# davelailai/DS-GCN

Hardware: AMD Instinct MI355X
Metric: clips/sec fwd+bwd, DS-STGCN NTU-60 3x64x25x2 (higher is better)
Workload: dtype f32; 1 GPU; DS-STGCN configs/dsstgcn/ntu60_xsub_3dkp/j.py (DSSTGCN_model.py kwargs), 64 clips/GPU of 3x64x25x2, 60 classes, train-mode BN, CE loss, fwd+bwd+grad all-reduce+SGD-nesterov per step; clips_per_gpu=64, global_batch=64, parallelism=dp1

## Files before the change

ds-gcn_amd/kernels.py:

```python
import contextlib
import sys

_active = None


def ops():
    return _active if _active is not None else sys.modules[__name__]


@contextlib.contextmanager
def use_ops(namespace):
    global _active
    prev = _active
    _active = namespace
    try:
        yield namespace
    finally:
        _active = prev


NAME = 'hip'

import torch

# ... 1394 lines not shown
    return KT or 3, types, c0s, bcs, dils, ws, bs


class _TemporalFused(torch.autograd.Function):

    @staticmethod
    def forward(ctx, z, zaug, scale, shift, coeff, gamma, beta, n_act, stride, KT, types, c0s, bcs, dils, eps, want_bn,
                bn, *wb):
        _require_cuda(z)
        ctx.bn, ctx.bn_in = bn, _bn_of(scale)
        z, zaug, scale, shift, coeff, gamma, beta = [_f32c(t) for t in (z, zaug, scale, shift, coeff, gamma, beta)]
        nbr = len(types)
        ws = [_f32c(t) for t in wb[:nbr]]
        bs = [_f32c(t) for t in wb[nbr:]]
        n, C, T, V = z.shape
        Tout = (T + stride - 1) // stride
        dev = z.device
        lib = native.lib()
        aug = zaug is not None
        tabs = (_int_array(types), _int_array(c0s), _int_array(bcs), _int_array(dils))
        rows = lib.dsgcn_tms_rows(0, n, C, T, V, stride, KT, nbr, tabs[0], tabs[2], tabs[3], int(aug))
        assert rows > 0
        f = torch.empty((n, C, Tout, V), device=dev, dtype=torch.float32)
        oaug = torch.empty((n, C, Tout), device=dev, dtype=torch.float32) if aug else None
        stats = torch.empty((rows, C, 2), device=dev, dtype=torch.float32) if want_bn else None
        rc = lib.dsgcn_tms_fwd(_ptr(z), _ptr(zaug), _ptr(scale), _ptr(shift), int(n_act), _ptr(coeff), _ptr(f),
                               _ptr(oaug), _ptr(stats), n, C, T, V, stride, KT, nbr, *tabs, _ptr_array(ws),
                               _ptr_array(bs), _stream())
        native.check(rc, 'dsgcn_tms_fwd')
        scale1 = shift1 = mean = var = None
        count = float(n * Tout * V)
        if want_bn:
            mean, var, scale1, shift1 = _finalize_stats(ctx, stats, rows, C, count, gamma, beta, eps, C)
        ctx.set_materialize_grads(False)
        ctx.save_for_backward(z, zaug, scale, shift, coeff, f, oaug, gamma, mean, var, *[w for w in ws if w is not None])
        ctx.cfg = (int(n_act), int(stride), int(KT), tuple(types), tuple(c0s), tuple(bcs), tuple(dils), float(eps),
                   bool(want_bn), count, beta is not None, tuple(b is not None for b in bs))
        ctx.defer_ok = _leafish(coeff, *wb)
        return f, scale1, shift1, mean, var

    @staticmethod
    def backward(ctx, gf, gscale, gshift, _gm, _gv):
        z, zaug, scale, shift, coeff, f, oaug, gamma, mean, var, *wsaved = ctx.saved_tensors
        n_act, stride, KT, types, c0s, bcs, dils, eps, want_bn, count, has_beta, has_b = ctx.cfg
        n, C, T, V = z.shape
        nbr = len(types)
        dev = z.device
        lib = native.lib()
        st = _stream()
        aug = zaug is not None
        gf, gscale, gshift = _f32c(gf), _f32c(gscale), _f32c(gshift)
        A0 = B0 = dgamma = dbeta = None
        if want_bn:
            dgamma, dbeta, A0, B0 = _bn_coef(ctx.bn, gscale, gshift, mean, var, gamma, eps, count, C, C)
        if gf is None:
            gf = torch.zeros_like(f)
        it = iter(wsaved)
        ws = [next(it) if t == 0 else None for t in types]
        tabs = (_int_array(types), _int_array(c0s), _int_array(bcs), _int_array(dils))
        rows = lib.dsgcn_tms_rows(1, n, C, T, V, stride, KT, nbr, tabs[0], tabs[2], tabs[3], int(aug))
        paff = torch.empty((rows, C, 2), device=dev, dtype=torch.float32)
        pcoeff = torch.empty((rows * nbr, V), device=dev, dtype=torch.float32) if aug else None
        dz = torch.empty_like(z)
        dzaug = torch.empty_like(zaug) if aug else None
        rc = lib.dsgcn_tms_dgrad(_ptr(z), _ptr(zaug), _ptr(scale), _ptr(shift), n_act, _ptr(coeff), _ptr(gf), _ptr(f),
                                 _ptr(A0), _ptr(B0), _ptr(oaug), _ptr(dz), _ptr(dzaug), _ptr(paff), _ptr(pcoeff), n, C, T,
                                 V, stride, KT, nbr, *tabs, _ptr_array(ws), st)
        native.check(rc, 'dsgcn_tms_dgrad')
        (dscale, dshift), _ = _affine_tail(paff, 2, [(scale, ctx.bn_in, 0, 1)])
        dcoeff = param_colsum(pcoeff, ctx.defer_ok) if aug else None
        dws, dbs = [None] * nbr, [None] * nbr
        if 0 in types:
            rows2 = lib.dsgcn_tms_rows(2, n, C, T, V, stride, KT, nbr, tabs[0], tabs[2], tabs[3], int(aug))
            part, dwp, dbp, pstride, split = _branch_partials(types, bcs, bcs, KT, rows2, dev, has_b)
            rc = lib.dsgcn_tms_wgrad(_ptr(z), _ptr(zaug), _ptr(scale), _ptr(shift), n_act, _ptr(coeff), _ptr(gf), _ptr(f),
                                     _ptr(A0), _ptr(B0), n, C, T, V, stride, KT, nbr, *tabs, dwp, dbp, pstride, st)
            native.check(rc, 'dsgcn_tms_wgrad')
            dws, dbs = split(param_colsum(part, ctx.defer_ok))
        dgamma, dbeta = _trim_affine_grads(dgamma, dbeta, gamma, has_beta)
        return (dz, dzaug, dscale, dshift, dcoeff, dgamma, dbeta, None, None, None, None, None, None, None, None, None,
                None, *dws, *dbs)


class _TemporalSplit(torch.autograd.Function):
    FRONT = 32

    @staticmethod
    def forward(ctx, z, zaug, scale, shift, coeff, gamma, beta, n_act, stride, types, c0s, bcs, dils, eps, want_bn, bn, *wb):
        _require_cuda(z)
        ctx.bn = bn
        z, zaug, scale, shift, coeff, gamma, beta = [_f32c(t) for t in (z, zaug, scale, shift, coeff, gamma, beta)]
        nbr = len(types)
        ws = [_f32c(t) for t in wb[:nbr]]
        bs = [_f32c(t) for t in wb[nbr:]]
        n, C, T, V = z.shape
        To = T // stride
        dev = z.device
        lib = native.lib()
        tabs = (_int_array(types), _int_array(c0s), _int_array(bcs), _int_array(dils))
        rows = lib.dsgcn_tms_split_rows(0, n, C, T, V, stride, 3, nbr, *tabs)
        assert rows > 0
        f = torch.empty((n, C, To, V), device=dev, dtype=torch.float32)
        oaug = torch.empty((n, C, To), device=dev, dtype=torch.float32)
        stats = torch.empty((rows, C, 2), device=dev, dtype=torch.float32) if want_bn else None
        rc = lib.dsgcn_tms_split_fwd(_ptr(z), _ptr(zaug), _ptr(scale), _ptr(shift), int(n_act), _ptr(coeff), _ptr(f),
                                     _ptr(oaug), _ptr(stats), n, C, T, V, stride, nbr, *tabs, _ptr_array(ws), _ptr_array(bs),
                                     _stream())
        native.check(rc, 'dsgcn_tms_split_fwd')
        scale1 = shift1 = mean = var = None
        count = float(n * To * V)
        if want_bn:
            mean, var, scale1, shift1 = _finalize_stats(ctx, stats, rows, C, count, gamma, beta, eps, C)
        ctx.set_materialize_grads(False)
        ctx.save_for_backward(z, zaug, scale, shift, coeff, f, oaug, gamma, mean, var, *[w for w in ws if w is not None])
        ctx.cfg = (int(n_act), int(stride), tuple(types), tuple(c0s), tuple(bcs), tuple(dils), float(eps), bool(want_bn),
                   count, beta is not None, tuple(b is not None for b in bs))
        ctx.bn_in = _bn_of(scale)
        ctx.defer_ok = _leafish(coeff, *wb)
        return f, scale1, shift1, mean, var

    @staticmethod
    def backward(ctx, gf, gscale, gshift, _gm, _gv):
        z, zaug, scale, shift, coeff, f, oaug, gamma, mean, var, *wsaved = ctx.saved_tensors
        n_act, stride, types, c0s, bcs, dils, eps, want_bn, count, has_beta, has_b = ctx.cfg
        n, C, T, V = z.shape
        To = f.shape[2]
        nbr = len(types)
        dev = z.device
        lib = native.lib()
        st = _stream()
        gf, gscale, gshift = _f32c(gf), _f32c(gscale), _f32c(gshift)
        A0 = B0 = dgamma = dbeta = None
        if want_bn:
            dgamma, dbeta, A0, B0 = _bn_coef(ctx.bn, gscale, gshift, mean, var, gamma, eps, count, C, C)
        FR = _TemporalSplit.FRONT
        gbuf = torch.empty(FR + f.numel() + FR + n * C * To, device=dev, dtype=torch.float32)
        ge = gbuf[FR:FR + f.numel()].view(f.shape)
        doaug = gbuf[2 * FR + f.numel():].view(n, C, To)
        pcoef = torch.empty((n * C, V), device=dev, dtype=torch.float32)
        rc = lib.dsgcn_tms_split_prep(_ptr(gf), _ptr(f), _ptr(oaug), _ptr(coeff), _ptr(A0), _ptr(B0), _ptr(ge), _ptr(doaug),
                                      _ptr(pcoef), n, C, To, V, st)
        native.check(rc, 'dsgcn_tms_split_prep')
        dcoeff = param_colsum(pcoef, ctx.defer_ok)
        it = iter(wsaved)
        ws = [next(it) if t == 0 else None for t in types]
        tabs = (_int_array(types), _int_array(c0s), _int_array(bcs), _int_array(dils))
        rows = lib.dsgcn_tms_split_rows(1, n, C, T, V, stride, 3, nbr, *tabs)
        part = torch.empty((rows, C, 2), device=dev, dtype=torch.float32)
        dz = torch.empty_like(z)
        dzaug = torch.empty_like(zaug)
        rc = lib.dsgcn_tms_split_dgrad(_ptr(z), _ptr(zaug), _ptr(scale), _ptr(shift), n_act, _ptr(ge), _ptr(doaug), _ptr(dz),
                                       _ptr(dzaug), _ptr(part), n, C, T, V, stride, nbr, *tabs, _ptr_array(ws), st)
        native.check(rc, 'dsgcn_tms_split_dgrad')
        (dscale, dshift), hosted = _affine_tail(part, 2, [(scale, ctx.bn_in, 0, 1)], launch=False)
        splits = lib.dsgcn_tms_split_rows(2, n, C, T, V, stride, 3, nbr, *tabs)
        wpart, dwp, dbp, pstride, split = _branch_partials(types, bcs, bcs, 3, splits, dev, has_b)
        rc = lib.dsgcn_tms_split_wgrad_jobs(_ptr(z), _ptr(zaug), _ptr(scale), _ptr(shift), n_act, _ptr(ge), _ptr(doaug), n, C,
                                            T, V, stride, nbr, *tabs, dwp, dbp, splits, pstride, *_job_array(hosted), st)
        native.check(rc, 'dsgcn_tms_split_wgrad_jobs')
        dws, dbs = split(param_colsum(wpart, ctx.defer_ok))
        dgamma, dbeta = _trim_affine_grads(dgamma, dbeta, gamma, has_beta)
        return (dz, dzaug, dscale, dshift, dcoeff, dgamma, dbeta, None, None, None, None, None, None, None, None, None,
                *dws, *dbs)


def _split_temporal(z, zaug, scale, shift, coeff, n_act, branch_cfg, widths, conv_w, conv_b, stride, gamma, beta, eps,
                    want_bn):
    if zaug is None or any(not isinstance(c, str) and c[0] != 'max' and c[0] != 3 for c in branch_cfg):
        return None
    if int(stride) != 1 and SPLIT_TEMPORAL == '1':
        return None
    KT, types, c0s, bcs, dils, ws, bs = _branch_tables(branch_cfg, widths, conv_w, conv_b)
    n, C, T, V = z.shape
    if native.lib().dsgcn_tms_split_rows(-1, n, C, T, V, int(stride), KT, len(types), _int_array(types), _int_array(c0s),
                                         _int_array(bcs), _int_array(dils)) != 1:
        return None
    bn = BNCtx() if want_bn else None
    out = _TemporalSplit.apply(z, zaug, scale, shift, coeff, gamma, beta, int(n_act), int(stride), types, c0s, bcs, dils,
                               float(eps), bool(want_bn), bn, *ws, *bs)
    if want_bn:
        _bn_attach(out[1], bn, out[3], out[4], gamma, eps, float(n * (T // int(stride)) * V), C)
    return out


def _fused_temporal(z, zaug, scale, shift, coeff, n_act, branch_cfg, widths, conv_w, conv_b, stride, gamma, beta, eps,
                    want_bn):
    KT, types, c0s, bcs, dils, ws, bs = _branch_tables(branch_cfg, widths, conv_w, conv_b)
    n, C, T, V = z.shape
    if FUSED_TEMPORAL == '0' or (FUSED_TEMPORAL == 'auto' and KT == 3):
        return None
    if sum(bcs) != C or any(c0s[i] + bcs[i] != c0s[i + 1] for i in range(len(bcs) - 1)) or c0s[0] != 0:
        return None
    rows = native.lib().dsgcn_tms_rows(0, n, C, T, V, int(stride), KT, len(types), _int_array(types), _int_array(bcs),
                                       _int_array(dils), int(zaug is not None))
    if rows <= 0:
        return None
    bn = BNCtx() if want_bn else None
    out = _TemporalFused.apply(z, zaug, scale, shift, coeff, gamma, beta, int(n_act), int(stride), KT, types, c0s, bcs,
                               dils, float(eps), bool(want_bn), bn, *ws, *bs)
    if want_bn:
        Tout = (T + int(stride) - 1) // int(stride)
        _bn_attach(out[1], bn, out[3], out[4], gamma, eps, float(n * Tout * V), C)
    return out


def temporal_ms(z, zaug, scale, shift, n_act, branch_cfg, widths, conv_w, conv_b, add_coeff, stride, gamma=None,
                beta=None, eps=1e-5, want_bn=False):
    _require_cuda(z)
    n, C, T, V = z.shape
    coeff = add_coeff if add_coeff.shape[0] == V else add_coeff[:V].contiguous()
    if FUSED_TEMPORAL != '0':
        out = _fused_temporal(z, zaug, scale, shift, coeff, n_act, branch_cfg, widths, conv_w, conv_b, stride, gamma, beta,
                              eps, want_bn)
        if out is not None:
            return out
    if SPLIT_TEMPORAL != '0':
        out = _split_temporal(z, zaug, scale, shift, coeff, n_act, branch_cfg, widths, conv_w, conv_b, stride, gamma, beta,
                              eps, want_bn)
        if out is not None:
            return out
    h = _BranchAct.apply(z, zaug, scale, shift, n_act)
    KT, types, c0s, bcs, dils, ws, bs = _branch_tables(branch_cfg, widths, conv_w, conv_b)
    o = _TapBranches.apply(h, int(stride), KT, C, types, c0s, c0s, bcs, bcs, dils, *ws, *bs)
    bn = BNCtx() if want_bn else None
    out = _TmsCombine.apply(o, coeff, gamma, beta, float(eps), bool(want_bn), bn)
    if want_bn:
        _bn_attach(out[1], bn, out[3], out[4], gamma, eps, float(o.shape[0] * o.shape[2] * (o.shape[3] - 1)), o.shape[1])
    return out


class _TapBranchesZero(_TapBranches):

    @staticmethod
    def forward(ctx, *args):
        return _TapBranches._run(ctx, torch.zeros, *args)

# ... 1025 lines not shown
```

include/dsgcn.h:

```cpp
#ifndef DSGCN_H_
#define DSGCN_H_

#include <stddef.h>
#include "dsgcn_jobs.h"
#ifdef __cplusplus
extern "C" {
#endif

#define DSGCN_EINVAL (-1)
#define DSGCN_EUNSUPPORTED (-2)

int dsgcn_version(void);

int dsgcn_set_matmul_precision(int level);
int dsgcn_get_matmul_precision(void);
int dsgcn_pwconv_terms(int dir, int n, int Ci, int Co, int T, int V, int stride);
int dsgcn_tconv_terms(int dir, int n, int Ci, int Co, int T, int V, int KT, int stride);

int dsgcn_aggregate_fwd(const float* zp, const float* scale, const float* shift, int relu, const float* ahat,
                        float* y, int n, int KC, int T, int V, void* stream);

int dsgcn_aggregate_bwd_partial_rows(int n, int T, int V);
int dsgcn_aggregate_bwd(const float* zp, const float* scale, const float* shift, int relu, const float* ahat,
                        const float* dy, float* dzp, float* dahat, float* partial, int n, int KC, int T, int V,
// ... 191 lines not shown
int dsgcn_tanhdiff_fwd(const float* proj, float* d, int n, int K, int R, int V, void* stream);
int dsgcn_tanhdiff_bwd_k(const float* d, const float* const* dd, float* dproj, int n, int K, int R, int V, void* stream);
int dsgcn_tanhdiff_aug_fwd(const float* proj, const float* A, float* d, int n, int K, int R, int V, void* stream);
int dsgcn_tanhdiff_aug_bwd(const float* d, const float* const* dd, float* dproj, float* dAp, int n, int K, int R, int V,
                           void* stream);
int dsgcn_ctr_wprep_multi(const dsgcn_ctr_prep_job* jobs, int njobs, void* stream);
int dsgcn_ctr_wfin_multi(const dsgcn_ctr_fin_job* jobs, int njobs, void* stream);
int dsgcn_ctr_affine_fwd(const float* const* s, const float* alpha, int alpha_stride, const float* A, const float* beta,
                         const float* G, float* ahat, int n, int K, int Co, int V, void* stream);
int dsgcn_ctr_affine_bwd(const float* const* s, const float* alpha, int alpha_stride, const float* dahat,
                         float* const* ds, float* prow, int n, int K, int Co, int V, void* stream);
int dsgcn_edge_select_fwd(const float* in, const int* edge_type, float* out, int n, int R, int E, int V, void* stream);
int dsgcn_edge_select_bwd(const float* dout, const int* edge_type, float* din, int n, int R, int E, int V, void* stream);
int dsgcn_plane_stats(const float* x, float* partial, long planes, int L, void* stream);

#define DSGCN_TYPED_MAX_TYPES 16
#define DSGCN_TYPED_MAX_PERIOD 1024
int dsgcn_typedconv_fwd(const float* x, const float* w, const float* b, const int* plan, int ntiles, float* y, int n,
                        int Ci, int Co, int TV, int L, int chunk, int P, void* stream);
int dsgcn_typedconv_dgrad(const float* dy, const float* w, const int* plan, int ntiles, float* dx, int n, int Ci, int Co,
                          int TV, int L, int chunk, int P, void* stream);
int dsgcn_typedconv_wgrad_rows(int n, int Ci, int Co, int P);
int dsgcn_typedconv_wgrad(const float* x, const float* dy, const int* plan, int ntiles, float* part, int n, int Ci, int Co,
                          int TV, int L, int chunk, int P, void* stream);

int dsgcn_add3(const float* a, const float* b, const float* c, float* out, long n, void* stream);

int dsgcn_pack(const float* const* src_table, const long* dst_offsets, const int* numels, int count, float* dst,
               void* stream);
int dsgcn_pack_fill(const float* const* src_table, const long* dst_offsets, const long* numels, int count, float* dst,
                    void* stream);

int dsgcn_dwcausal_fwd(const float* h, const float* w, const float* b, const int* dil, float* y, int n, int C, int T,
                       int V, int stride, int KM, void* stream);
int dsgcn_dwcausal_bwd(const float* h, const float* w, const int* dil, const float* dy, float* dh, float* part, int n,
                       int C, int T, int V, int stride, int KM, void* stream);

int dsgcn_mlpwin_supported(int n, int C, int T, int V1, int stride, int KM, int nwin, const int* type, const int* c0,
                           const int* width, const int* dil, const int* add);
int dsgcn_mlpwin_partial_stride(int C, int KM, int nwin, const int* type, const int* width);
int dsgcn_mlpwin_fwd(const float* h, const float* o, float* u, const float* tapw, const float* tapb, int n, int C, int T,
                     int V1, int stride, int KM, int nwin, const int* type, const int* c0, const int* width, const int* dil,
                     const int* add, const float* const* w1, const float* const* b1, void* stream);
int dsgcn_mlpwin_bwd(const float* h, const float* o, const float* du, const float* tapw, const float* tapb, float* dh,
                     float* dout, float* gbuf, float* part, int n, int C, int T, int V1, int stride, int KM, int nwin, const int* type,
                     const int* c0, const int* width, const int* dil, const int* add, const float* const* w1, int pstride,
                     void* stream);

int dsgcn_tms_rows(int which, int n, int C, int T, int V, int stride, int KT, int nbr, const int* type, const int* bc,
                   const int* dil, int aug);
int dsgcn_tms_fwd(const float* z, const float* zaug, const float* scale, const float* shift, int n_act,
                  const float* coeff, float* f, float* oaug, float* stats, int n, int C, int T, int V, int stride, int KT,
                  int nbr, const int* type, const int* c0, const int* bc, const int* dil, const float* const* w,
                  const float* const* b, void* stream);
int dsgcn_tms_dgrad(const float* z, const float* zaug, const float* scale, const float* shift, int n_act,
                    const float* coeff, const float* gf, const float* f, const float* A0, const float* B0,
                    const float* oaug, float* dz, float* dzaug, float* paff, float* pcoeff, int n, int C, int T, int V,
                    int stride, int KT, int nbr, const int* type, const int* c0, const int* bc, const int* dil,
                    const float* const* w, void* stream);
int dsgcn_tms_wgrad(const float* z, const float* zaug, const float* scale, const float* shift, int n_act,
                    const float* coeff, const float* gf, const float* f, const float* A0, const float* B0, int n, int C,
                    int T, int V, int stride, int KT, int nbr, const int* type, const int* c0, const int* bc,
                    const int* dil, float* const* dwp, float* const* dbp, int pstride, void* stream);

int dsgcn_tms_split_rows(int which, int n, int C, int T, int V, int stride, int KT, int nbr, const int* type,
                         const int* c0, const int* bc, const int* dil);
int dsgcn_tms_split_fwd(const float* z, const float* zaug, const float* scale, const float* shift, int n_act,
                        const float* coeff, float* f, float* oaug, float* stats, int n, int C, int T, int V, int stride,
                        int nbr, const int* type, const int* c0, const int* bc, const int* dil, const float* const* w,
                        const float* const* b, void* stream);
int dsgcn_tms_split_prep(const float* gf, const float* f, const float* oaug, const float* coeff, const float* A0,
                         const float* B0, float* ge, float* doaug, float* pcoef, int n, int C, int T, int V,
                         void* stream);
int dsgcn_tms_split_dgrad(const float* z, const float* zaug, const float* scale, const float* shift, int n_act,
                          const float* ge, const float* doaug, float* dz, float* dzaug, float* part, int n, int C, int T,
                          int V, int stride, int nbr, const int* type, const int* c0, const int* bc, const int* dil,
                          const float* const* w, void* stream);
int dsgcn_tms_split_wgrad_jobs(const float* z, const float* zaug, const float* scale, const float* shift, int n_act,
                               const float* ge, const float* doaug, int n, int C, int T, int V, int stride, int nbr,
                               const int* type, const int* c0, const int* bc, const int* dil, float* const* dwp,
                               float* const* dbp, int splits, int pstride, const dsgcn_bn_coef_job* jobs, int njobs,
                               void* stream);

int dsgcn_gate_fwd(const float* y, const float* g, int mode, float* out, float* rout, int rmode, int n, int C, int T,
                   int V, void* stream);
int dsgcn_gate_bwd(const float* y, const float* g, int mode, const float* gout, const float* drout, int rmode, float* dy,
                   float* dgp, int n, int C, int T, int V, void* stream);

int dsgcn_skeleton_prep(const float* raw, const long* offset, const int* M, const int* T, const int* flags,
                        const int* f0, const int* f1, const float* center, const float* matrix, const int* parent,
                        float* out, int N, int clips, int Mout, int clip_len, int V, int C, int nfeat, int fmask,
                        int scored, int loop, void* stream);

int dsgcn_skeleton_prep_streams(const float* raw, const long* offset, const int* M, const int* T, const int* flags,
                                const int* f0, const int* f1, const float* center, const float* matrix,
                                const int* parent, float* const* out, int N, int clips, int Mout, int clip_len, int V,
                                int C, int nfeat, int fmask, int scored, int loop, void* stream);

int dsgcn_head_loss_fwd(const float* feat, const float* w, const float* b, const long long* label, int N, int M, int C,
                        int K, float loss_weight, float* pooled, float* score, float* prob, float* clip, float* loss,
                        double* acc, void* stream);
int dsgcn_head_loss_bwd(const float* prob, const float* pooled, const float* w, const long long* label, const float* gloss,
                        int N, int M, int C, int K, float loss_weight, float* dfeat, float* dw, float* db, void* stream);

int dsgcn_head_target_fwd(const float* feat, const float* w, const float* b, const float* class_weight, const void* target,
                          int mode, int N, int M, int C, int K, float loss_weight, float* pooled, float* score,
                          float* dscore, float* clip, float* loss, float* den, double* acc, void* stream);
int dsgcn_head_target_bwd(const float* dscore, const float* pooled, const float* w, const float* gloss, const float* den,
                          int N, int M, int C, int K, float loss_weight, float* dfeat, float* dw, float* db, void* stream);

int dsgcn_head_test_fwd(const float* feat, const float* w, const float* b, int N, int clips, int M, int C, int K, int mode,
                        float* clip_score, float* out, void* stream);

int dsgcn_head_ensemble_fwd(const float* const* feat, const float* const* w, const float* const* b, const float* weight,
                            int S, int N, int clips, int M, int C, int K, int mode, float* stream_out, float* out,
                            void* stream);

int dsgcn_feat_ext_fwd(const float* x, const float* w, const float* b, int videos, int clips, int M, int C, int T, int V,
                       int K, int pool_mask, float* out32, void* out16, void* stream);

int dsgcn_graph_pool_splits(int videos, int group, int K, int mid, int V);
int dsgcn_graph_pool(const float* ahat, float* out, float* ws, int videos, int group, int K, int mid, int V, int L,
                     int layer, void* stream);

int dsgcn_bn_running_multi(float* const* running_mean, float* const* running_var, const float* const* mean,
                           const float* const* var, long long* const* num_batches_tracked, const int* C,
                           const float* unbias, const float* momentum, int njobs, void* stream);

int dsgcn_data_bn_fwd(const float* x, const float* gamma, const float* beta, float* running_mean, float* running_var,
                      long long* num_batches_tracked, float* y, float* save_mean, float* save_invstd, float* scratch,
                      int N, int M, int T, int V, int C, int mvc, int training, float eps, float momentum,
                      void* stream);
int dsgcn_data_bn_bwd(const float* x, const float* dy, const float* save_mean, const float* save_invstd, float* pg,
                      float* pb, int N, int M, int T, int V, int C, int mvc, void* stream);

int dsgcn_sgd_step(float* p, const float* g, float* buf, const float* lr, float momentum, float weight_decay,
                   int nesterov, long long n, void* stream);

int dsgcn_grad_norm_rows(long long n);
int dsgcn_grad_norm_partials(const float* g, long long n, int norm_type, double* partial, void* stream);
int dsgcn_sgd_step_clip(float* p, float* g, float* buf, const float* lr, const double* partial, int rows, int norm_type,
                        float max_norm, float* grad_norm_out, float momentum, float weight_decay, int nesterov,
                        long long n, void* stream);

int dsgcn_grad_accum(float* acc, const float* g, long long n, void* stream);
int dsgcn_grad_accum_finish(float* acc, float* g, const float* factor, long long n, void* stream);

#define DSGCN_OPTIM_SKIP (-1)
int dsgcn_optim_chunks(long long n);
int dsgcn_optim_table(const int* ends, const int* group, int ntens, const double* wd, int groups, long long n, int* first);
int dsgcn_sgd_group_step(float* p, float* g, float* buf, const int* ends, const int* group, const int* first, int ntens,
                         const double* lr, const double* wd, int groups, float momentum, int nesterov, long long n,
                         void* stream);
int dsgcn_sgd_group_step_clip(float* p, float* g, float* buf, const int* ends, const int* group, const int* first, int ntens,
                              const double* lr, const double* wd, int groups, const double* partial, int rows,
                              int norm_type, float max_norm, float* grad_norm_out, float momentum, int nesterov,
                              long long n, void* stream);
int dsgcn_adam_step(float* p, float* g, float* m, float* v, int* step, const int* ends, const int* group, const int* first,
                    int ntens, const double* lr, const double* wd, int groups, double beta1, double beta2, float eps,
                    int decoupled, long long n, void* stream);
int dsgcn_adam_step_clip(float* p, float* g, float* m, float* v, int* step, const int* ends, const int* group,
                         const int* first, int ntens, const double* lr, const double* wd, int groups, const double* partial,
                         int rows, int norm_type, float max_norm, float* grad_norm_out, double beta1, double beta2,
                         float eps, int decoupled, long long n, void* stream);

int dsgcn_sgd_step_hyper(float* p, const float* g, float* buf, const float* lr, const double* hyper, float weight_decay,
// ... 24 lines not shown
```

Measured before the change: 6118 clips/s.

## Add MFMA-based fused temporal-split kernel for narrow branches in forward and dgrad

Adds a new HIP kernel family (tsp16) that computes the multi-branch temporal split convolution for branches up to 16 channels. It uses 16x16x4 f32 MFMA with permlane swaps, folds the BN affine, ReLU and augmented coefficient into the operand load, and fuses BN statistics or dgrad partial sums into the epilogue. Pool and elementwise branches run in the same launch. Python dispatches to it by default when a cached shape check passes, falling back to the old kernels otherwise. The change adds substantial hand-written assembly and indexing complexity, with new correctness risk at boundaries.

```diff
diff --git a/ds-gcn_amd/csrc/tsp16.hip b/ds-gcn_amd/csrc/tsp16.hip
--- /dev/null
+++ b/ds-gcn_amd/csrc/tsp16.hip
@@ -0,0 +1,762 @@
+#include <algorithm>
+
+#include "common.h"
+
+namespace {
+
+constexpr int T16_NT = 256;
+constexpr int T16_MAXBR = 8;
+constexpr int T16_H = 4;
+constexpr int T16_ROWS = 16;
+constexpr size_t T16_LDS_BLOCK = 40000;
+constexpr size_t T16_LDS_MAX = 64 * 1024;
+
+struct T16Branch {
+  int type;
+  int c0, bc, dil;
+  const float* w;
+  const float* b;
+};
+
+struct T16Args {
+  const float* z; const float* zaug; const float* scale; const float* shift;
+  const float* coeff;
+  float* f; float* oaug; float* stats;
+  const float* ge; const float* doaug;
+  float* dz; float* dzaug; float* part;
+  int n_act, n, C, T, V, nbr, ngrp, ngrpa, nconv, eplanes, sboff, haw, ppb;
+  int cw[T16_MAXBR];
+  T16Branch br[T16_MAXBR];
+};
+
+__device__ __forceinline__ void t16_store4(f32x4 v, __amdgpu_buffer_rsrc_t r, int voff) {
+  __builtin_amdgcn_raw_buffer_store_b128(__builtin_bit_cast(u32x4v, v), r, voff, 0, 0);
+}
+__device__ __forceinline__ int t16_cp(int bc) { return (min(T16_ROWS, max(bc, 1)) + 7) & ~7; }
+
+__device__ __forceinline__ void t16_kslots(f32x4& x, f32x4& y) {
+  float x0 = x[0], x1 = x[1], x2 = x[2], x3 = x[3], y0 = y[0], y1 = y[1], y2 = y[2], y3 = y[3];
+  asm volatile(
+      "s_nop 1\n\t"
+      "v_permlane32_swap_b32 %0, %4\n\t"
+      "v_permlane32_swap_b32 %1, %5\n\t"
+      "v_permlane32_swap_b32 %2, %6\n\t"
+      "v_permlane32_swap_b32 %3, %7\n\t"
+      "v_permlane16_swap_b32 %0, %4\n\t"
+      "v_permlane16_swap_b32 %1, %5\n\t"
+      "v_permlane16_swap_b32 %2, %6\n\t"
+      "v_permlane16_swap_b32 %3, %7\n\t"
+      "s_nop 1"
+      : "+v"(x0), "+v"(x1), "+v"(x2), "+v"(x3), "+v"(y0), "+v"(y1), "+v"(y2), "+v"(y3));
+  x = f32x4{x0, x1, x2, x3};
+  y = f32x4{y0, y1, y2, y3};
+}
+
+template <bool FWD, bool ODD, bool AUG>
+__device__ __forceinline__ void t16_conv(const T16Args& a, const T16Branch& br, bool first, float* lds, int grp, int lane, int wave) {
+  constexpr int KT = 3, PDK = 2, NS = KT * PDK;
+  constexpr bool FOLD = FWD && !AUG;
+  const int tid = threadIdx.x;
+  const int half = lane >> 5, l31 = lane & 31;
+  const int g4 = lane >> 4, c16 = lane & 15;
+  const int V = AUG ? 1 : a.V, C = a.C, bc = br.bc;
+  const int T = a.T;
+  const int L = T * V, L4 = L * 4;
+  const int CP = t16_cp(bc), S = KT * CP + 1;
+  float* Ws = lds;
+  f32x2v* SB = reinterpret_cast<f32x2v*>(lds + a.sboff);
+  float* BI = lds + a.sboff + 2 * T16_ROWS;
+  float* HA = lds + a.sboff + 3 * T16_ROWS;
+  const int HAW = a.haw;
+  const bool relu = br.c0 < a.n_act;
+  const int wt = grp * 4 + wave;
+  const long total = (long)a.n * L;
+  const bool wlive = (long)wt * 128 < total;
+  const int g0 = wlive ? wt * 128 : 0;
+  const int n0 = g0 / L;
+  auto locate = [&](int l, int& pp, int& dd) -> bool {
+    pp = g0 - n0 * L + 4 * l;
+    dd = 0;
+    while (pp >= L) { pp -= L; ++dd; }
+    return wlive && n0 + dd < a.n;
+  };
+  int p, ds;
+  const bool pok = locate(l31, p, ds);
+  const float* srcp = FWD ? (AUG ? a.zaug : a.z) : (AUG ? a.doaug : a.ge);
+  const __amdgpu_buffer_rsrc_t rs = buf_rsrc(srcp, (size_t)a.n * C * L * 4);
+  const int rowbase = ((n0 + ds) * C + br.c0 + half) * L;
+  int t0 = 0, v0 = 0;
+  bool nx[4] = {false, false, false, false};
+  if constexpr (FOLD) {
+    divmod_small(p, V, 1.f / (float)V, t0, v0);
+#pragma unroll
+    for (int k = 0; k < 4; ++k) nx[k] = v0 + k >= V;
+  }
+  const int sh = (FWD ? br.dil : -br.dil) * V;
+  int vP[KT][2];
+  float mk[KT][4];
+  bool fS[KT][2], fE[KT][2];
+#pragma unroll
+  for (int tap = 0; tap < KT; ++tap)
+#pragma unroll
+    for (int j = 0; j < 2; ++j) {
+      const int q = p + (tap - 1) * sh + 2 * j;
+      const bool e0 = q >= 0 && q < L, e1 = q + 1 >= 0 && q + 1 < L;
+      const bool s = ODD && !e0 && e1, e = ODD && e0 && !e1;
+      const int qa = s ? q + 1 : (e ? q - 1 : q);
+      fS[tap][j] = s;
+      fE[tap][j] = e;
+      vP[tap][j] = (pok && (e0 || e1)) ? (rowbase + qa) * 4 : BUF_OOB;
+      mk[tap][2 * j] = (pok && e0) ? 1.f : 0.f;
+      mk[tap][2 * j + 1] = (pok && e1) ? 1.f : 0.f;
+    }
+  auto load = [&](int tap, int ks) -> f32x4 {
+    const int soff = 2 * ks * L4;
+    if (tap == 1) return buf_load<4>(rs, vP[1][0], soff);
+    const f32x2v lo = buf_load<2>(rs, vP[tap][0], soff), hi = buf_load<2>(rs, vP[tap][1], soff);
+    return f32x4{lo.x, lo.y, hi.x, hi.y};
+  };
+
+  float cf[4] = {0.f, 0.f, 0.f, 0.f};
+  int gl = 0;
+  const int Gs = (grp * 512) / V - T16_H;
+  if constexpr (FOLD) {
+#pragma unroll
+    for (int k = 0; k < 4; ++k) cf[k] = a.coeff[nx[k] ? v0 + k - V : v0 + k];
+    gl = pok ? (n0 + ds) * T + t0 - Gs : T16_H;
+  }
+  const int KS2 = ((bc + 3) >> 2) << 1;
+  f32x4 buf[NS];
+#pragma unroll
+  for (int u = 0; u < NS; ++u) {
+    buf[u] = load(u % KT, u / KT);
+    __builtin_amdgcn_sched_barrier(0);
+  }
+  {
+    const int run = bc * KT, wtotal = bc * run;
+    float wv[3], hv[FOLD ? 8 : 1];
+#pragma unroll
+    for (int q = 0; q < 3; ++q) {
+      const int i = tid + q * T16_NT;
+      wv[q] = i < wtotal ? br.w[i] : 0.f;
+    }
+    f32x2v sb = {0.f, 0.f};
+    float bi = 0.f;
+    if (tid < bc) {
+      const int c = br.c0 + tid;
+      sb = f32x2v{a.scale ? a.scale[c] : 1.f, a.shift ? a.shift[c] : 0.f};
+      if (br.b) bi = br.b[tid];
+    }
+    const int hsh = 31 - __builtin_clz(HAW);
+    const int he = tid & (HAW - 1), hc0 = tid >> hsh, hcs = T16_NT >> hsh;
+    const int hG = Gs + he, hn = hG / T, ht = hG - hn * T;
+    const bool hok = hG >= 0 && hn < a.n;
+    const float* hsrc = a.zaug + ((size_t)(hok ? hn : 0) * C + br.c0) * T + (hok ? ht : 0);
+    if constexpr (FOLD) {
+#pragma unroll
+      for (int q = 0; q < 8; ++q) {
+        const int ci = hc0 + q * hcs;
+        hv[q] = (hok && ci < bc) ? hsrc[(size_t)ci * T] : 0.f;
+      }
+    }
+    {
+      f32x4* w4 = reinterpret_cast<f32x4*>(Ws);
+      for (int i = tid; i < (T16_ROWS * S) >> 2; i += T16_NT) w4[i] = f32x4{0.f, 0.f, 0.f, 0.f};
+    }
+    const float invrun = 1.f / (float)run;
+    auto wat = [&](int i) -> int {
+      int co, r;
+      divmod_small(i, run, invrun, co, r);
+      const int ci = (r * 43691) >> 17, tap = r - ci * KT;
+      return co * S + tap * CP + ci;
+    };
+    if (tid < T16_ROWS) {
+      SB[tid] = sb;
+      BI[tid] = bi;
+    }
+    __syncthreads();
+#pragma unroll
+    for (int q = 0; q < 3; ++q) {
+      const int i = tid + q * T16_NT;
+      if (i < wtotal) Ws[wat(i)] = wv[q];
+    }
+    if constexpr (FOLD) {
+#pragma unroll
+      for (int q = 0; q < 8; ++q) {
+        const int ci = hc0 + q * hcs;
+        if (ci < T16_ROWS) {
+          const f32x2v e = SB[ci];
+          float y = fmaf(hv[q], e.x, e.y);
+          if (relu) y = fmaxf(y, 0.f);
+          HA[ci * HAW + he] = (hok && ci < bc) ? y : 0.f;
+        }
+      }
+    }
+    __syncthreads();
+  }
+  f32x4 acc[4][2];
+#pragma unroll
+  for (int q = 0; q < 4; ++q)
+#pragma unroll
+    for (int h = 0; h < 2; ++h) acc[q][h] = f32x4{0.f, 0.f, 0.f, 0.f};
+  int aoff[KT];
+#pragma unroll
+  for (int pi = 0; pi < KT; ++pi) {
+    const int u = 2 * pi + (g4 >> 1), tap = u % KT, kl = 2 * (u / KT) + (g4 & 1);
+    aoff[pi] = FWD ? c16 * S + tap * CP + kl : kl * S + tap * CP + c16;
+  }
+  const int astep = FWD ? 2 * PDK : 2 * PDK * S;
+  auto hfrag = [&](int tap, int ks) -> f32x2v {
+    const float* hp = HA + (2 * ks + half) * HAW + gl + (tap - 1) * br.dil;
+    return f32x2v{hp[0], hp[1]};
+  };
+  const int kmax = T16_ROWS / 2 - 1;
+  f32x2v sbv[2], hab[2];
+  float av = Ws[aoff[0]];
+  sbv[0] = SB[half];
+  if constexpr (FOLD) hab[0] = hfrag(0, 0);
+  const float* Wb = Ws;
+  for (int base = 0; base < KS2; base += PDK) {
+    f32x4 bb[2];
+#pragma unroll
+    for (int u = 0; u < NS; ++u) {
+      const int tap = u % KT, ks = base + u / KT;
+      const int cur = u & 1, nxt = cur ^ 1;
+      const int tn = (u + 1) % KT, kn = min(base + (u + 1) / KT, kmax);
+      if (FWD) sbv[nxt] = SB[2 * kn + half];
+      if constexpr (FOLD) hab[nxt] = hfrag(tn, kn);
+      f32x4 b = buf[u];
+      if (tap != 1) {
+        if (ODD) {
+          const float x0 = b.x, y0 = b.y, x1 = b.z, y1 = b.w;
+          b.x = fE[tap][0] ? y0 : x0;
+          b.y = fS[tap][0] ? x0 : y0;
+          b.z = fE[tap][1] ? y1 : x1;
+          b.w = fS[tap][1] ? x1 : y1;
+        }
+      }
+      if (FWD) {
+#pragma unroll
+        for (int q = 0; q < 4; ++q) {
+          float v = fmaf(b[q], sbv[cur].x, sbv[cur].y);
+          if (relu) v = fmaxf(v, 0.f);
+          if constexpr (FOLD) v = fmaf(nx[q] ? hab[cur].y : hab[cur].x, cf[q], v);
+          if (tap != 1) v *= mk[tap][q];
+          b[q] = v;
+        }
+      } else if (ODD && tap != 1) {
+#pragma unroll
+        for (int q = 0; q < 4; ++q) b[q] *= mk[tap][q];
+      }
+      bb[cur] = b;
+      if (cur == 1) {
+        const int pi = u >> 1;
+        const float a0 = av;
+        av = pi + 1 < KT ? Wb[aoff[pi + 1]] : (base + PDK < KS2 ? Wb[astep + aoff[0]] : Ws[aoff[0]]);
+        __builtin_amdgcn_sched_barrier(0);
+        t16_kslots(bb[0], bb[1]);
+#pragma unroll
+        for (int q = 0; q < 4; ++q) {
+          acc[q][0] = __builtin_amdgcn_mfma_f32_16x16x4f32(a0, bb[0][q], acc[q][0], 0, 0, 0);
+          acc[q][1] = __builtin_amdgcn_mfma_f32_16x16x4f32(a0, bb[1][q], acc[q][1], 0, 0, 0);
+        }
+        __builtin_amdgcn_sched_barrier(0);
+        buf[u - 1] = load((u - 1) % KT, min(base + (u - 1) / KT + PDK, KS2 - 1));
+        buf[u] = load(tap, min(ks + PDK, KS2 - 1));
+        __builtin_amdgcn_sched_barrier(0);
+      }
+    }
+    Wb += astep;
+  }
+  float* Tw = lds + wave * (T16_ROWS * 36);
+  int ooff[2];
+  bool oko[2];
+  float cfo[2][4];
+#pragma unroll
+  for (int h = 0; h < 2; ++h) {
+    int po, dso;
+    oko[h] = locate(16 * h + c16, po, dso);
+    ooff[h] = oko[h] ? (((n0 + dso) * C + br.c0) * L + po) * 4 : BUF_OOB;
+#pragma unroll
+    for (int k = 0; k < 4; ++k) cfo[h][k] = 0.f;
+    if constexpr (FOLD) {
+      int to, vo;
+      divmod_small(po, V, 1.f / (float)V, to, vo);
+#pragma unroll
+      for (int k = 0; k < 4; ++k) cfo[h][k] = a.coeff[vo + k >= V ? vo + k - V : vo + k];
+    }
+  }
+  if constexpr (FWD) {
+    double* Ss = reinterpret_cast<double*>(lds + 4 * T16_ROWS * 36);
+    const __amdgpu_buffer_rsrc_t ro = buf_rsrc(AUG ? a.oaug : a.f, (size_t)a.n * C * L4);
+    const bool stats = !AUG && a.stats != nullptr;
+    __syncthreads();
+    float sq[2][4];
+#pragma unroll
+    for (int h = 0; h < 2; ++h) {
+#pragma unroll
+      for (int r = 0; r < 4; ++r) {
+        const int ch = 4 * g4 + r;
+        const float bias = BI[ch];
+        f32x4 val;
+        float s = 0.f, qq = 0.f;
+#pragma unroll
+        for (int k = 0; k < 4; ++k) {
+          val[k] = fmaf(bias, 1.f + cfo[h][k], acc[k][h][r]);
+          s += val[k];
+          qq = fmaf(val[k], val[k], qq);
+        }
+        t16_store4(val, ro, buf_rowoff(ch < bc, ooff[h], ch * L4));
+        if (stats) {
+          const bool ok = ch < bc && oko[h];
+          Tw[ch * 36 + 16 * h + c16] = ok ? s : 0.f;
+          sq[h][r] = ok ? qq : 0.f;
+        }
+      }
+    }
+    if (stats) {
+      wave_lds_sync();
+      float sf = tile36_rowsum<float>(Tw, half, c16);
+      wave_lds_sync();
+#pragma unroll
+      for (int h = 0; h < 2; ++h)
+#pragma unroll
+        for (int r = 0; r < 4; ++r) Tw[(4 * g4 + r) * 36 + 16 * h + c16] = sq[h][r];
+      wave_lds_sync();
+      float qf = tile36_rowsum<float>(Tw, half, c16);
+      wave_lds_sync();
+      sf += __shfl_xor(sf, 32, 64);
+      qf += __shfl_xor(qf, 32, 64);
+      if (lane < T16_ROWS) {
+        Ss[(wave * T16_ROWS + lane) * 2 + 0] = (double)sf;
+        Ss[(wave * T16_ROWS + lane) * 2 + 1] = (double)qf;
+      }
+      __syncthreads();
+      if (tid < bc) {
+        double s4 = 0.0, q4 = 0.0;
+#pragma unroll
+        for (int w = 0; w < 4; ++w) { s4 += Ss[(w * T16_ROWS + tid) * 2]; q4 += Ss[(w * T16_ROWS + tid) * 2 + 1]; }
+        a.stats[((size_t)grp * C + br.c0 + tid) * 2 + 0] = (float)s4;
+        a.stats[((size_t)grp * C + br.c0 + tid) * 2 + 1] = (float)q4;
+      }
+    }
+  } else {
+    float* Ss = lds + 4 * T16_ROWS * 36;
+    const __amdgpu_buffer_rsrc_t rx = buf_rsrc(AUG ? a.zaug : a.z, (size_t)a.n * C * L4);
+    const __amdgpu_buffer_rsrc_t ro = buf_rsrc(AUG ? a.dzaug : a.dz, (size_t)a.n * C * L4);
+    f32x4 xa[2][4];
+#pragma unroll
+    for (int h = 0; h < 2; ++h)
+#pragma unroll
+      for (int r = 0; r < 4; ++r) {
+        const int ch = 4 * g4 + r;
+        xa[h][r] = buf_load<4>(rx, buf_rowoff(ch < bc, ooff[h], ch * L4), 0);
+      }
+    __builtin_amdgcn_sched_barrier(0);
+    __syncthreads();
+    float su[2][4];
+#pragma unroll
+    for (int h = 0; h < 2; ++h) {
+#pragma unroll
+      for (int r = 0; r < 4; ++r) {
+        const int ch = 4 * g4 + r;
+        const f32x2v e = SB[ch];
+        float u0 = 0.f, u1 = 0.f;
+        f32x4 d;
+#pragma unroll
+        for (int q = 0; q < 4; ++q) {
+          const float x = xa[h][r][q];
+          const float pre = fmaf(x, e.x, e.y);
+          const float dv = (!relu || pre > 0.f) ? acc[q][h][r] : 0.f;
+          d[q] = dv * e.x;
+          u0 = fmaf(dv, x, u0);
+          u1 += dv;
+        }
+        t16_store4(d, ro, buf_rowoff(ch < bc, ooff[h], ch * L4));
+        const bool ok = ch < bc && oko[h];
+        Tw[ch * 36 + 16 * h + c16] = ok ? u0 : 0.f;
+        su[h][r] = ok ? u1 : 0.f;
+      }
+    }
+    wave_lds_sync();
+    float s0 = tile36_rowsum<float>(Tw, half, c16);
+    wave_lds_sync();
+#pragma unroll
+    for (int h = 0; h < 2; ++h)
+#pragma unroll
+      for (int r = 0; r < 4; ++r) Tw[(4 * g4 + r) * 36 + 16 * h + c16] = su[h][r];
+    wave_lds_sync();
+    float s1 = tile36_rowsum<float>(Tw, half, c16);
+    wave_lds_sync();
+    s0 += __shfl_xor(s0, 32, 64);
+    s1 += __shfl_xor(s1, 32, 64);
+    if (lane < T16_ROWS) {
+      Ss[(wave * T16_ROWS + lane) * 2 + 0] = s0;
+      Ss[(wave * T16_ROWS + lane) * 2 + 1] = s1;
+    }
+    __syncthreads();
+    const size_t prow = (size_t)(AUG ? a.ngrp + a.n + grp : grp) * C;
+    if (tid < bc) {
+      float v0s = 0.f, v1s = 0.f;
+#pragma unroll
+      for (int w = 0; w < 4; ++w) { v0s += Ss[(w * T16_ROWS + tid) * 2]; v1s += Ss[(w * T16_ROWS + tid) * 2 + 1]; }
+      a.part[(prow + br.c0 + tid) * 2 + 0] = v0s;
+      a.part[(prow + br.c0 + tid) * 2 + 1] = v1s;
+    }
+  }
+  float* tab = FWD ? (AUG ? nullptr : a.stats) : a.part;
+  if (tab && first) {
+    const size_t trow = (size_t)((!FWD && AUG) ? a.ngrp + a.n + grp : grp) * C;
+    for (int i = 0; i < a.nbr; ++i)
+      if (a.br[i].type != 0)
+        for (int k = tid; k < a.br[i].bc * 2; k += T16_NT) tab[(trow + a.br[i].c0) * 2 + k] = 0.f;
+  }
+}
+
+constexpr int T16_PQ = 8;
+
+template <bool FWD>
+__device__ __forceinline__ void t16_elem(const T16Args& a, const T16Branch& br, float* lw, int n, int c, int lane) {
+  const int V = a.V, T = a.T, L = T * V, L4n = L >> 2, C = a.C;
+  const int cc = br.c0 + c;
+  const size_t plane = (size_t)n * C + cc;
+  const bool relu = cc < a.n_act;
+  const bool pool = br.type == 1;
+  const float invV = 1.f / (float)V;
+  const int Tp = (T + 3) & ~3;
+  float* hp = lw;
+  float* gp = lw + L;
+  float* ha = lw + (FWD ? 1 : 2) * L;
+  float* oa = ha + Tp;
+  float* cf = oa + Tp;
+  const float* za = a.zaug + plane * T;
+  const f32x4* z4 = reinterpret_cast<const f32x4*>(a.z + plane * L);
+  const f32x4* g4 = FWD ? nullptr : reinterpret_cast<const f32x4*>(a.ge + plane * L);
+  auto act = [&](float x, float s, float b) -> float {
+    const float y = fmaf(x, s, b);
+    return relu ? fmaxf(y, 0.f) : y;
+  };
+  const float s = a.scale ? a.scale[cc] : 1.f, b = a.shift ? a.shift[cc] : 0.f;
+  f32x4 zr[T16_PQ], gr[FWD ? 1 : T16_PQ];
+#pragma unroll
+  for (int q = 0; q < T16_PQ; ++q) {
+    const int i = min(q * 64 + lane, L4n - 1);
+    zr[q] = z4[i];
+    if (!FWD) gr[q] = g4[i];
+  }
+  float zav[2], gav[2];
+#pragma unroll
+  for (int q = 0; q < 2; ++q) {
+    const int t = lane + 64 * q;
+    zav[q] = za[min(t, T - 1)];
+    gav[q] = FWD ? 0.f : a.doaug[plane * T + min(t, T - 1)];
+  }
+  const float cfv = FWD ? a.coeff[min(lane, V - 1)] : 0.f;
+  if (pool) {
+    f32x4* h4 = reinterpret_cast<f32x4*>(hp);
+    f32x4* gl4 = reinterpret_cast<f32x4*>(gp);
+#pragma unroll
+    for (int q = 0; q < T16_PQ; ++q) {
+      const int i = q * 64 + lane;
+      if (i < L4n) {
+        f32x4 v = zr[q];
+        if (FWD) {
+#pragma unroll
+          for (int k = 0; k < 4; ++k) v[k] = act(v[k], s, b);
+        }
+        h4[i] = v;
+        if (!FWD) gl4[i] = gr[q];
+      }
+    }
+  }
+#pragma unroll
+  for (int q = 0; q < 2; ++q) {
+    const int t = lane + 64 * q;
+    if (t < T) {
+      ha[t] = act(zav[q], s, b);
+      if (!FWD) oa[t] = gav[q];
+    }
+  }
+  for (int t = lane + 128; t < T; t += 64) {
+    ha[t] = act(za[t], s, b);
+    if (!FWD) oa[t] = a.doaug[plane * T + t];
+  }
+  if (FWD && lane < V) cf[lane] = cfv;
+  wave_lds_sync();
+  if constexpr (FWD) {
+    for (int t = lane; t < T; t += 64) {
+      float v = ha[t];
+      if (pool) {
+        if (t >= 1) v = fmaxf(v, ha[t - 1]);
+        if (t + 1 < T) v = fmaxf(v, ha[t + 1]);
+      }
+      a.oaug[plane * T + t] = v;
+    }
+    f32x4* fp = reinterpret_cast<f32x4*>(a.f + plane * L);
+    double sv = 0.0, qv = 0.0;
+    if (pool) {
+      float* fo = a.f + plane * L;
+      for (int e = lane; e < L; e += 64) {
+        int t, v;
+        divmod_small(e, V, invV, t, v);
+        float x = hp[e], o = ha[t];
+        if (t >= 1) { x = fmaxf(x, hp[e - V]); o = fmaxf(o, ha[t - 1]); }
+        if (t + 1 < T) { x = fmaxf(x, hp[e + V]); o = fmaxf(o, ha[t + 1]); }
+        const float r = fmaf(o, cf[v], x);
+        fo[e] = r;
+        sv += (double)r;
+        qv = fma((double)r, (double)r, qv);
+      }
+    } else
+#pragma unroll
+    for (int q = 0; q < T16_PQ; ++q) {
+      const int i = q * 64 + lane;
+      if (i < L4n) {
+        int t, v;
+        divmod_small(4 * i, V, invV, t, v);
+        float r[4];
+#pragma unroll
+        for (int k = 0; k < 4; ++k) {
+          const float x = act(zr[q][k], s, b);
+          const float o = ha[t];
+          r[k] = fmaf(o, cf[v], x);
+          if (++v == V) { v = 0; ++t; }
+        }
+        fp[i] = f32x4{r[0], r[1], r[2], r[3]};
+        const float s4 = (r[0] + r[1]) + (r[2] + r[3]);
+        const float q4 = fmaf(r[0], r[0], r[1] * r[1]) + fmaf(r[2], r[2], r[3] * r[3]);
+        sv += (double)s4;
+        qv += (double)q4;
+      }
+    }
+    if (a.stats) {
+      sv = wave_sum_d(sv);
+      qv = wave_sum_d(qv);
+      if (lane == 0) {
+        a.stats[((size_t)(a.ngrp + n) * C + cc) * 2 + 0] = (float)sv;
+        a.stats[((size_t)(a.ngrp + n) * C + cc) * 2 + 1] = (float)qv;
+      }
+    }
+  } else {
+    auto route = [&](const float* hcol, const float* gcol, int t, int st) -> float {
+      auto row = [&](int r) -> float { return (r >= 0 && r < T) ? act(hcol[r * st], s, b) : -INFINITY; };
+      const float v = act(hcol[t * st], s, b);
+      const float m2 = row(t - 2), m1 = row(t - 1), p1 = row(t + 1), p2 = row(t + 2);
+      float g = 0.f;
+      if (t >= 1 && v > m2 && v > m1) g += gcol[(t - 1) * st];
+      if (v > m1 && v >= p1) g += gcol[t * st];
+      if (t + 1 < T && v >= p1 && v >= p2) g += gcol[(t + 1) * st];
+      return g;
+    };
+    f32x4* dp = reinterpret_cast<f32x4*>(a.dz + plane * L);
+    float u0 = 0.f, u1 = 0.f;
+    if (pool) {
+      float* dzo = a.dz + plane * L;
+      for (int e = lane; e < L; e += 64) {
+        int t, v;
+        divmod_small(e, V, invV, t, v);
+        const float x = hp[e];
+        float g = route(hp + v, gp + v, t, V);
+        if (relu && !(fmaf(x, s, b) > 0.f)) g = 0.f;
+        dzo[e] = g * s;
+        u0 = fmaf(g, x, u0);
+        u1 += g;
+      }
+    } else
+#pragma unroll
+    for (int q = 0; q < T16_PQ; ++q) {
+      const int i = q * 64 + lane;
+      if (i < L4n) {
+        float r[4];
+#pragma unroll
+        for (int k = 0; k < 4; ++k) {
+          const float x = zr[q][k];
+          float g = gr[q][k];
+          if (relu && !(fmaf(x, s, b) > 0.f)) g = 0.f;
+          r[k] = g * s;
+          u0 = fmaf(g, x, u0);
+          u1 += g;
+        }
+        dp[i] = f32x4{r[0], r[1], r[2], r[3]};
+      }
+    }
+    auto route1 = [&](int t) -> float {
+      if (!pool) return oa[t];
+      auto row = [&](int r) -> float { return (r >= 0 && r < T) ? ha[r] : -INFINITY; };
+      const float v = ha[t];
+      const float m2 = row(t - 2), m1 = row(t - 1), p1 = row(t + 1), p2 = row(t + 2);
+      float g = 0.f;
+      if (t >= 1 && v > m2 && v > m1) g += oa[t - 1];
+      if (v > m1 && v >= p1) g += oa[t];
+      if (t + 1 < T && v >= p1 && v >= p2) g += oa[t + 1];
+      return g;
+    };
+    for (int t = lane; t < T; t += 64) {
+      const float x = t < 128 ? zav[t >> 6] : za[t];
+      float g = route1(t);
+      if (relu && !(fmaf(x, s, b) > 0.f)) g = 0.f;
+      a.dzaug[plane * T + t] = g * s;
+      u0 = fmaf(g, x, u0);
+      u1 += g;
+    }
+    u0 = wave_sum(u0);
+    u1 = wave_sum(u1);
+    if (lane == 0) {
+      a.part[((size_t)(a.ngrp + n) * C + cc) * 2 + 0] = u0;
+      a.part[((size_t)(a.ngrp + n) * C + cc) * 2 + 1] = u1;
+    }
+  }
+}
+
+template <bool FWD>
+__global__ __launch_bounds__(T16_NT, 4) void k_tsp16(T16Args a) {
+  extern __shared__ __attribute__((aligned(16))) float lds[];
+  const int lane = threadIdx.x & 63;
+  const int wave = __builtin_amdgcn_readfirstlane(threadIdx.x >> 6);
+  const int cb = a.nconv * a.ngrp, cba = a.nconv * a.ngrpa, b = blockIdx.x;
+  if (b < cb) {
+    const int w = b % a.nconv, grp = b / a.nconv;
+    const T16Branch& br = a.br[a.cw[w]];
+    if ((br.dil * a.V) & 1) t16_conv<FWD, true, false>(a, br, w == 0, lds, grp, lane, wave);
+    else t16_conv<FWD, false, false>(a, br, w == 0, lds, grp, lane, wave);
+    return;
+  }
+  if (b < cb + cba) {
+    const int w = (b - cb) % a.nconv, grp = (b - cb) / a.nconv;
+    const T16Branch& br = a.br[a.cw[w]];
+    if (br.dil & 1) t16_conv<FWD, true, true>(a, br, w == 0, lds, grp, lane, wave);
+    else t16_conv<FWD, false, true>(a, br, w == 0, lds, grp, lane, wave);
+    return;
+  }
+  if (wave >= a.ppb) return;
+  const int pl = (b - cb - cba) * a.ppb + wave;
+  if (pl >= a.n * a.eplanes) return;
+  const int n = pl / a.eplanes;
+  int c = pl - n * a.eplanes;
+  float* tab = FWD ? a.stats : a.part;
+  if (c == 0 && tab) {
+    for (int i = 0; i < a.nbr; ++i)
+      if (a.br[i].type == 0)
+        for (int k = lane; k < a.br[i].bc * 2; k += 64) tab[((size_t)(a.ngrp + n) * a.C + a.br[i].c0) * 2 + k] = 0.f;
+  }
+  const int per = (FWD ? 1 : 2) * a.T * a.V + 2 * ((a.T + 3) & ~3) + 32;
+  for (int i = 0; i < a.nbr; ++i) {
+    if (a.br[i].type == 0) continue;
+    if (c < a.br[i].bc) {
+      t16_elem<FWD>(a, a.br[i], lds + (size_t)wave * per, n, c, lane);
+      return;
+    }
+    c -= a.br[i].bc;
+  }
+}
+
+int t16_fill(T16Args& a, bool fwd, size_t* ldsb, int n, int C, int T, int V, int stride, int KT, int nbr, const int* type,
+             const int* c0, const int* bc, const int* dil) {
+  if (n <= 0 || C <= 0 || T <= 0 || V <= 0 || nbr <= 0 || nbr > T16_MAXBR || !type || !c0 || !bc || !dil) return DSGCN_EINVAL;
+  a.n = n; a.C = C; a.T = T; a.V = V; a.nbr = nbr;
+  int nconv = 0, eplanes = 0, wmax = 0, next = 0;
+  for (int i = 0; i < nbr; ++i) {
+    T16Branch& b = a.br[i];
+    b.type = type[i]; b.c0 = c0[i]; b.bc = bc[i]; b.dil = dil[i];
+    if (b.bc <= 0 || b.c0 != next) return b.bc <= 0 ? DSGCN_EINVAL : 0;
+    next += b.bc;
+    if (b.type == 0) {
+      a.cw[nconv] = i;
+      ++nconv;
+      wmax = std::max(wmax, b.bc);
+      if (b.dil < 1 || b.dil > T16_H) return 0;
+    } else if (b.type == 1 || b.type == 2) {
+      eplanes += b.bc;
+    } else {
+      return DSGCN_EINVAL;
+    }
+  }
+  if (next != C) return 0;
+  if (KT != 3 || stride != 1 || nconv == 0 || wmax > T16_ROWS || (V & 1) == 0 || V < 5 || V > 25 || T % 4 ||
+      (long)T * V > 2048)
+    return 0;
+  const long L = (long)T * V;
+  if ((long)n * C * L * 4 >= (1L << 31) - 4096 || (long)n * L >= (1L << 31) - 256) return 0;
+  if (n > 32768) return 0;
+  a.nconv = nconv;
+  a.eplanes = eplanes;
+  a.haw = 32;
+  while (a.haw < 511 / V + 2 + 2 * T16_H + 3) a.haw *= 2;
+  a.ngrp = (int)(((long)n * T * V + 511) / 512);
+  a.ngrpa = (int)(((long)n * T + 511) / 512);
+  const size_t wsf = (size_t)T16_ROWS * (3 * T16_ROWS + 1);
+  const size_t epf = (size_t)4 * T16_ROWS * 36 + (size_t)4 * T16_ROWS * 2 * 2;
+  const size_t convf = (std::max(wsf, epf) + 3) & ~(size_t)3;
+  a.sboff = (int)convf;
+  const size_t convb = (convf + 3 * T16_ROWS + (fwd ? (size_t)T16_ROWS * a.haw : 0)) * sizeof(float);
+  const size_t per = ((size_t)(fwd ? 1 : 2) * T * V + 2 * ((T + 3) & ~3) + 32) * sizeof(float);
+  a.ppb = 4;
+  while (a.ppb > 1 && a.ppb * per > T16_LDS_BLOCK) a.ppb >>= 1;
+  *ldsb = std::max(convb, eplanes ? a.ppb * per : (size_t)0);
+  return *ldsb <= T16_LDS_MAX ? 1 : 0;
+}
+
+template <bool FWD>
+int t16_launch(T16Args& a, size_t lds, hipStream_t st) {
+  const long blocks = (long)a.nconv * (a.ngrp + a.ngrpa) + ((long)a.n * a.eplanes + a.ppb - 1) / a.ppb;
+  if (blocks <= 0 || blocks >= (1L << 31)) return DSGCN_EUNSUPPORTED;
+  hipLaunchKernelGGL((k_tsp16<FWD>), dim3((unsigned)blocks), dim3(T16_NT), lds, st, a);
+  DSGCN_LAUNCH_CHECK();
+  return 0;
+}
+
+}
+
+extern "C" {
+
+int dsgcn_tsp16_rows(int which, int n, int C, int T, int V, int stride, int KT, int nbr, const int* type, const int* c0,
+                     const int* bc, const int* dil) {
+  T16Args a = {};
+  size_t lf = 0, lb = 0;
+  if (t16_fill(a, true, &lf, n, C, T, V, stride, KT, nbr, type, c0, bc, dil) <= 0) return 0;
+  if (t16_fill(a, false, &lb, n, C, T, V, stride, KT, nbr, type, c0, bc, dil) <= 0) return 0;
+  if (which == -1) return 1;
+  if (which == 0) return a.ngrp + n;
+  if (which == 1) return a.ngrp + n + a.ngrpa;
+  return 0;
+}
+
+int dsgcn_tsp16_fwd(const float* z, const float* zaug, const float* scale, const float* shift, int n_act,
+                    const float* coeff, float* f, float* oaug, float* stats, int n, int C, int T, int V, int stride,
+                    int nbr, const int* type, const int* c0, const int* bc, const int* dil, const float* const* w,
+                    const float* const* b, void* stream) {
+  if (!z || !zaug || !coeff || !f || !oaug || !w) return DSGCN_EINVAL;
+  T16Args a = {};
+  size_t lds = 0;
+  const int ok = t16_fill(a, true, &lds, n, C, T, V, stride, 3, nbr, type, c0, bc, dil);
+  if (ok < 0) return ok;
+  if (ok == 0) return DSGCN_EUNSUPPORTED;
+  a.z = z; a.zaug = zaug; a.scale = scale; a.shift = shift; a.n_act = n_act; a.coeff = coeff;
+  a.f = f; a.oaug = oaug; a.stats = stats;
+  for (int i = 0; i < nbr; ++i) {
+    a.br[i].w = w[i]; a.br[i].b = b ? b[i] : nullptr;
+    if (type[i] == 0 && !a.br[i].w) return DSGCN_EINVAL;
+  }
+  return t16_launch<true>(a, lds, (hipStream_t)stream);
+}
+
+int dsgcn_tsp16_dgrad(const float* z, const float* zaug, const float* scale, const float* shift, int n_act,
+                      const float* ge, const float* doaug, float* dz, float* dzaug, float* part, int n, int C, int T,
+                      int V, int stride, int nbr, const int* type, const int* c0, const int* bc, const int* dil,
+                      const float* const* w, void* stream) {
+  if (!z || !zaug || !ge || !doaug || !dz || !dzaug || !part || !w) return DSGCN_EINVAL;
+  T16Args a = {};
+  size_t lds = 0;
+  const int ok = t16_fill(a, false, &lds, n, C, T, V, stride, 3, nbr, type, c0, bc, dil);
+  if (ok < 0) return ok;
+  if (ok == 0) return DSGCN_EUNSUPPORTED;
+  a.z = z; a.zaug = zaug; a.scale = scale; a.shift = shift; a.n_act = n_act;
+  a.ge = ge; a.doaug = doaug; a.dz = dz; a.dzaug = dzaug; a.part = part;
+  for (int i = 0; i < nbr; ++i) {
+    a.br[i].w = w[i];
+    if (type[i] == 0 && !a.br[i].w) return DSGCN_EINVAL;
+  }
+  return t16_launch<false>(a, lds, (hipStream_t)stream);
+}
+
+}
diff --git a/ds-gcn_amd/kernels.py b/ds-gcn_amd/kernels.py
--- a/ds-gcn_amd/kernels.py
+++ b/ds-gcn_amd/kernels.py
@@ -1500,6 +1500,18 @@
                 None, *dws, *dbs)
 
 
+TSP16 = int(_os.environ.get('DSGCN_TSP16', '3'))
+_tsp16_shapes = {}
+
+
+def _tsp16_takes(lib, n, C, T, V, stride, types, c0s, bcs, dils):
+    key = (n, C, T, V, stride, tuple(types), tuple(c0s), tuple(bcs), tuple(dils))
+    if key not in _tsp16_shapes:
+        _tsp16_shapes[key] = lib.dsgcn_tsp16_rows(-1, n, C, T, V, stride, 3, len(types), _int_array(types), _int_array(c0s),
+                                                  _int_array(bcs), _int_array(dils)) == 1
+    return _tsp16_shapes[key]
+
+
 class _TemporalSplit(torch.autograd.Function):
     FRONT = 32
 
@@ -1521,10 +1533,11 @@
         f = torch.empty((n, C, To, V), device=dev, dtype=torch.float32)
         oaug = torch.empty((n, C, To), device=dev, dtype=torch.float32)
         stats = torch.empty((rows, C, 2), device=dev, dtype=torch.float32) if want_bn else None
-        rc = lib.dsgcn_tms_split_fwd(_ptr(z), _ptr(zaug), _ptr(scale), _ptr(shift), int(n_act), _ptr(coeff), _ptr(f),
-                                     _ptr(oaug), _ptr(stats), n, C, T, V, stride, nbr, *tabs, _ptr_array(ws), _ptr_array(bs),
-                                     _stream())
-        native.check(rc, 'dsgcn_tms_split_fwd')
+        name = 'dsgcn_tsp16_fwd' if (TSP16 & 1) and _tsp16_takes(lib, n, C, T, V, stride, types, c0s, bcs, dils) else 'dsgcn_tms_split_fwd'
+        rc = getattr(lib, name)(_ptr(z), _ptr(zaug), _ptr(scale), _ptr(shift), int(n_act), _ptr(coeff), _ptr(f),
+                                _ptr(oaug), _ptr(stats), n, C, T, V, stride, nbr, *tabs, _ptr_array(ws), _ptr_array(bs),
+                                _stream())
+        native.check(rc, name)
         scale1 = shift1 = mean = var = None
         count = float(n * To * V)
         if want_bn:
@@ -1567,9 +1580,10 @@
         part = torch.empty((rows, C, 2), device=dev, dtype=torch.float32)
         dz = torch.empty_like(z)
         dzaug = torch.empty_like(zaug)
-        rc = lib.dsgcn_tms_split_dgrad(_ptr(z), _ptr(zaug), _ptr(scale), _ptr(shift), n_act, _ptr(ge), _ptr(doaug), _ptr(dz),
-                                       _ptr(dzaug), _ptr(part), n, C, T, V, stride, nbr, *tabs, _ptr_array(ws), st)
-        native.check(rc, 'dsgcn_tms_split_dgrad')
+        name = 'dsgcn_tsp16_dgrad' if (TSP16 & 2) and _tsp16_takes(lib, n, C, T, V, stride, types, c0s, bcs, dils) else 'dsgcn_tms_split_dgrad'
+        rc = getattr(lib, name)(_ptr(z), _ptr(zaug), _ptr(scale), _ptr(shift), n_act, _ptr(ge), _ptr(doaug), _ptr(dz),
+                                _ptr(dzaug), _ptr(part), n, C, T, V, stride, nbr, *tabs, _ptr_array(ws), st)
+        native.check(rc, name)
         (dscale, dshift), hosted = _affine_tail(part, 2, [(scale, ctx.bn_in, 0, 1)], launch=False)
         splits = lib.dsgcn_tms_split_rows(2, n, C, T, V, stride, 3, nbr, *tabs)
         wpart, dwp, dbp, pstride, split = _branch_partials(types, bcs, bcs, 3, splits, dev, has_b)
diff --git a/include/dsgcn.h b/include/dsgcn.h
--- a/include/dsgcn.h
+++ b/include/dsgcn.h
@@ -297,6 +297,17 @@
                                float* const* dbp, int splits, int pstride, const dsgcn_bn_coef_job* jobs, int njobs,
                                void* stream);
 
+int dsgcn_tsp16_rows(int which, int n, int C, int T, int V, int stride, int KT, int nbr, const int* type, const int* c0,
+                     const int* bc, const int* dil);
+int dsgcn_tsp16_fwd(const float* z, const float* zaug, const float* scale, const float* shift, int n_act,
+                    const float* coeff, float* f, float* oaug, float* stats, int n, int C, int T, int V, int stride,
+                    int nbr, const int* type, const int* c0, const int* bc, const int* dil, const float* const* w,
+                    const float* const* b, void* stream);
+int dsgcn_tsp16_dgrad(const float* z, const float* zaug, const float* scale, const float* shift, int n_act,
+                      const float* ge, const float* doaug, float* dz, float* dzaug, float* part, int n, int C, int T,
+                      int V, int stride, int nbr, const int* type, const int* c0, const int* bc, const int* dil,
+                      const float* const* w, void* stream);
+
 int dsgcn_gate_fwd(const float* y, const float* g, int mode, float* out, float* rout, int rmode, int n, int C, int T,
                    int V, void* stream);
 int dsgcn_gate_bwd(const float* y, const float* g, int mode, const float* gout, const float* drout, int rmode, float* dy,
```

Result: no change. 6171 clips/s, median of 6 (+0.9%).
